# Deci-AI/super-gradients

Measured on NVIDIA H100. Metric: images/sec YOLO-NAS-S 640 bf16 train, higher is better.
Workload: dtype bf16

## Files before the change

include/sgb200.h:

```cpp
#ifndef SGB200_H_
#define SGB200_H_

#include <stdint.h>

#ifdef __cplusplus
extern "C" {
#endif

#define SGB_OK 0
#define SGB_E_INVALID (-1)
#define SGB_E_UNSUPPORTED (-2)
#define SGB_E_CUDA (-3)
#define SGB_E_ARCH (-4)

#define SGB_ACT_NONE 0
#define SGB_ACT_RELU 1
#define SGB_ACT_SILU 2

typedef uint16_t sgb_bf16;

typedef struct SgbConvDesc {
  int32_t N, H, W, C;
  int32_t K, R, S;
  int32_t P, Q;
  int32_t stride, pad;
  int32_t x_pitch, x_off;
  int32_t y_pitch, y_off;
  int32_t up2;
  int32_t centre_from;
} SgbConvDesc;

typedef struct SgbEpilogue {
  const float* scale;
  const float* shift;
  const sgb_bf16* residual;
  double* stats;
  int32_t stats_repl;
  int32_t act;
  int32_t out_f32;
} SgbEpilogue;

const char* sgb_last_error(void);
int sgb_version(void);
int sgb_check_device(void);
int64_t sgb_sm100_launches(void);
int64_t sgb_conv_halo_launches(void);
void sgb_conv_force_im2col(int on);

int sgb_conv_fprop(const SgbConvDesc* d, const sgb_bf16* x, const sgb_bf16* w_krsc, void* y, const SgbEpilogue* ep,
                   void* stream);
int sgb_conv_dgrad(const SgbConvDesc* d, const sgb_bf16* dy, const sgb_bf16* w_crsk, sgb_bf16* dx, int accumulate,
                   void* stream);
int sgb_conv_wgrad(const SgbConvDesc* d, const sgb_bf16* x, const sgb_bf16* dy, float* dw_krsc, void* stream);
int sgb_weight_prepare(const float* w_oihw, int K, int C, int R, int S, int c_pad, sgb_bf16* w_krsc, sgb_bf16* w_crsk,
                       const float* scale, int add_identity, void* stream);
int sgb_wgrad_to_oihw(const float* dw_krsc, int K, int C, int R, int S, int c_pad, float* g_oihw, int accumulate,
                      void* stream);
typedef struct SgbWeightItem {
  const float* w;
  const float* scale;
  sgb_bf16* krsc;
  sgb_bf16* crsk;
  int32_t K, C, R, S, c_pad, add_identity;
  int32_t kp, koff, etaps, etap;
  int64_t start;
} SgbWeightItem;
typedef struct SgbWgradItem {
  const float* dw;
  float* g;
  int32_t K, C, R, S, c_pad, accumulate;
  int64_t start;
} SgbWgradItem;
int sgb_weight_prepare_batch(const SgbWeightItem* items_dev, int n_items, int64_t total, void* stream);
typedef struct SgbAlphaItem {
  const float* dw1;
  const float* w1;
  const float* alpha;
  const float* dab;
  const float* bias1;
  float* g_w1;
  float* g_bias;
  float* g_alpha;
  int32_t K, C, c_pad, pad_;
} SgbAlphaItem;
int sgb_qarep_alpha_finish_batch(const SgbAlphaItem* items_dev, int n_items, void* stream);
int sgb_wgrad_to_oihw_batch(const SgbWgradItem* items_dev, int n_items, int64_t total, void* stream);
int sgb_convt2x2_fprop(const SgbConvDesc* d, const sgb_bf16* x_small, const sgb_bf16* w_up, const float* bias,
                       sgb_bf16* y_up, void* stream);

int sgb_nchw_f32_to_nhwc_bf16(const float* x, int N, int C, int H, int W, sgb_bf16* y, int y_pitch, int y_off, int c_out,
                              void* stream);
int sgb_stem_patches_f32(const float* x, int N, int C, int H, int W, int R, int stride, int pad, sgb_bf16* y, int P, int Q, int c_out,
                         void* stream);
int sgb_nhwc_bf16_to_nchw_f32(const sgb_bf16* x, int N, int C, int H, int W, int x_pitch, int x_off, float* y,
                              void* stream);

typedef struct SgbBnDesc {
  int64_t M;
  int32_t C;
  int32_t x_pitch, x_off;
// ... 305 lines not shown
```

super_gradients_b200/csrc/capi.cu:

```cuda
#include <cstdarg>
#include <cstdio>

#include "common.cuh"
#include "conv_sm100.h"
#include "sm100_host.h"

static thread_local char g_err[512] = "";

void sgb_set_error(const char* fmt, ...) {
  va_list ap;
  va_start(ap, fmt);
  vsnprintf(g_err, sizeof(g_err), fmt, ap);
  va_end(ap);
}

int sgb_cuda_check(cudaError_t e, const char* what) {
  if (e == cudaSuccess) return SGB_OK;
  sgb_set_error("%s: %s", what, cudaGetErrorString(e));
  return SGB_E_CUDA;
}

extern "C" const char* sgb_last_error(void) { return g_err; }
extern "C" int sgb_version(void) { return 100; }
extern "C" int sgb_check_device(void) {
  int dev = 0;
  if (int rc = sgb_cuda_check(cudaGetDevice(&dev), "cudaGetDevice")) return rc;
  cudaDeviceProp prop;
  if (int rc = sgb_cuda_check(cudaGetDeviceProperties(&prop, dev), "cudaGetDeviceProperties")) return rc;
  if (prop.major != 9) {
    sgb_set_error("libsgb200 is built for sm_90a only; device is sm_%d%d", prop.major, prop.minor);
    return SGB_E_ARCH;
  }
  return SGB_OK;
}

extern "C" int64_t sgb_sm100_launches(void) { return (int64_t)sm100::launch_count(); }
extern "C" int64_t sgb_conv_halo_launches(void) { return (int64_t)sm100::halo_launch_count(); }
extern "C" void sgb_conv_force_im2col(int on) { sm100::force_im2col(on != 0); }
```

super_gradients_b200/csrc/conv_sm100.cu:

```cuda
#include <cuda.h>

#include <cstdlib>
#include <cstring>

#include "common.cuh"
#include "conv_sm100.h"
#include "sm100_host.h"
#include "sm100_ptx.cuh"

namespace sm100 {

constexpr int BLOCK_M = 128;
constexpr int NUM_THREADS = 384;
constexpr int CONSUMER_THREADS = 256;
constexpr int MAX_STAGES = 8;

struct Params {
  int M;
  int N;
  int C;
  int KC;
  int n_tiles;
  int stages;
  int P, Q;
// ... 335 lines not shown
      int t = off > 0 ? 0 : CENTRE_TAP;
      uint32_t sa_t = sa + (uint32_t)((t / 3) * HALO_W + t % 3) * 16u, sb_t = sb + (uint32_t)(p.tap_b[t] * ksteps) * b_box;
      for (int k = 0, ks = 0, nk = 8 * off + ksteps; k < nk; ++k) {
        const uint64_t da = smem_desc_noswizzle(sa_t + (uint32_t)(2 * ks) * HALO_CG_BYTES, HALO_CG_BYTES, HALO_W * 16);
        const uint64_t db = smem_desc(sb_t + (uint32_t)ks * b_box, 32, 16u, 256u);
        mma_kk<BN>(acc, da, db, k != 0);
        if (++ks == (t == CENTRE_TAP ? ksteps : off) && ++t < 9) {
          ks = 0;
          sa_t = sa + (uint32_t)((t / 3) * HALO_W + t % 3) * 16u;
          sb_t = sb + (uint32_t)(p.tap_b[t] * ksteps) * b_box;
        }
      }
      wgmma_commit();
      wgmma_wait<0>();
      fence_regs(acc);
      __syncwarp();
      if (lane == 0) mbar_arrive(empty_bar(stg));

      const int n_img = mt / p.halo_thw;
      const int rem = mt - n_img * p.halo_thw;
      const int th = rem / p.halo_tw, tw = rem - th * p.halo_tw;
      const int ow = tw * HALO_TILE + (lane >> 2);
      long long orow[2];
      bool row_ok[2];
#pragma unroll
      for (int h = 0; h < 2; ++h) {
        const int oh = th * HALO_TILE + 2 * wq + h;
        row_ok[h] = oh < p.P && ow < p.Q;
        orow[h] = row_ok[h] ? ((long long)n_img * p.P + oh) * p.Q + ow : 0;
      }
      tile_epilogue<BN, 4>(p, acc, orow, row_ok, nt, wg, wq, lane, s_part + wg * 4 * 2 * BN, s_stats + wg * 2 * p.N);
    }
  }
  __syncthreads();
  if (p.stats) {
    for (int i = threadIdx.x; i < 2 * p.N; i += NUM_THREADS) s_stats[i] += s_stats[2 * p.N + i];
    __syncthreads();
  }
  flush_stats(p, s_stats);
}

struct WParams {
  int K, C;
  int R, S, stride, pad, P, Q;
  int npix;
  int CB;
  int n_ctiles;
  int rb_all, rb_off;
  int items;
  int pix_per_cta;
  int stages;
  int cpad;
  float* dw;
};
constexpr int WPIX = 64;

__host__ __device__ __forceinline__ int wgrad_row_blocks(const WParams& p, int tap) {
  return p.R * p.S == 9 && tap != CENTRE_TAP ? p.rb_off : p.rb_all;
}

template <int NB>
__global__ void __launch_bounds__(NUM_THREADS, 1)
wgrad_wgmma_kernel(const __grid_constant__ CUtensorMap map_dy, const __grid_constant__ CUtensorMap map_x, const WParams p) {
  SGB_GRID_DEP_LAUNCH();
  extern __shared__ __align__(1024) unsigned char smem_raw[];
  const uint32_t smem_base = (smem_u32(smem_raw) + 1023u) & ~1023u;
  const uint32_t a_bytes = 2 * WPIX * 128;
  const uint32_t b_box = WPIX * p.CB * 2;
  const int boxes = NB / p.CB;
  const uint32_t stage_bytes = a_bytes + (uint32_t)boxes * b_box;
  const uint32_t ctrl = smem_base + p.stages * stage_bytes;
  auto full_bar = [&](int s) { return ctrl + 8u * s; };
  auto empty_bar = [&](int s) { return ctrl + 8u * (MAX_STAGES + s); };

  const int warp = threadIdx.x >> 5, lane = threadIdx.x & 31;
  int w = blockIdx.x;
  const int split = w / (p.items * p.n_ctiles);
  w -= split * p.items * p.n_ctiles;
  int tap = 0, tap_items = (wgrad_row_blocks(p, 0) + 1) / 2;
  while (w >= tap_items * p.n_ctiles) {
    w -= tap_items * p.n_ctiles;
    tap_items = (wgrad_row_blocks(p, ++tap) + 1) / 2;
  }
  const int ctile = w / tap_items, item = w - ctile * tap_items;
  const bool shared_rows = 2 * item + 1 == wgrad_row_blocks(p, tap);
  const int row0 = 128 * item;
  const int pix0 = split * p.pix_per_cta;
  const int pix1 = min(pix0 + p.pix_per_cta, p.npix);
  const int n_iters = (pix1 - pix0 + WPIX - 1) / WPIX;

  if (threadIdx.x == 0) {
    for (int s = 0; s < p.stages; ++s) {
      mbar_init(full_bar(s), 1);
      mbar_init(empty_bar(s), shared_rows ? 4 : 8);
    }
    asm volatile("fence.mbarrier_init.release.cluster;" ::: "memory");
    asm volatile("fence.proxy.async.shared::cta;" ::: "memory");
  }
  __syncthreads();
  SGB_GRID_DEP_WAIT();

  if (n_iters > 0) {
    if (warp == 0) {
      if (elect_one()) {
        const int pq = p.P * p.Q;
        const int r = tap / p.S, s = tap - r * p.S;
// ... 18 lines not shown
            par ^= 1;
          }
        }
      }
    } else if (warp >= 4) {
      const int wg = (warp >> 2) - 1, wq = warp & 3;
      const int b_row_bytes = p.CB * 2;
      float acc[NB / 2];
      const int it0 = shared_rows ? wg : 0, it_step = shared_rows ? 2 : 1;
      const uint32_t a_off = shared_rows ? 0u : (uint32_t)wg * (WPIX * 128);
      int stg = it0, prev = -1;
      uint32_t par = 0;
      for (int it = it0; it < n_iters; it += it_step) {
        mbar_wait(full_bar(stg), par);
        const uint32_t sa = smem_base + stg * stage_bytes + a_off, sb = smem_base + stg * stage_bytes + a_bytes;
        wgmma_fence();
#pragma unroll
        for (int j = 0; j < WPIX / 16; ++j) {
          const uint64_t da = smem_desc(sa + (uint32_t)j * 16u * 128u, 128, WPIX * 128, 8 * 128);
          const uint64_t db = smem_desc(sb + (uint32_t)j * 16u * (uint32_t)b_row_bytes, b_row_bytes, b_box, 8u * (uint32_t)b_row_bytes);
          mma_mn<NB>(acc, da, db, (it != it0 || j != 0) ? 1u : 0u);
        }
        wgmma_commit();
        if (prev >= 0) {
          wgmma_wait<1>();
          __syncwarp();
          if (lane == 0) mbar_arrive(empty_bar(prev));
        }
        prev = stg;
        if ((stg += it_step) >= p.stages) {
          stg -= p.stages;
          par ^= 1;
        }
      }
      if (prev < 0) return;
      wgmma_wait<0>();
      fence_regs(acc);
      const int row_len = p.R * p.S * p.cpad;
#pragma unroll
      for (int h = 0; h < 2; ++h) {
        const int ko = row0 + (shared_rows ? 0 : wg * 64) + wq * 16 + (lane >> 2) + 8 * h;
        if (ko < p.K) {
          float* drow = p.dw + (long long)ko * row_len + tap * p.cpad + ctile * NB + 2 * (lane & 3);
#pragma unroll
          for (int j = 0; j < NB / 8; ++j)
            asm volatile("red.global.add.v2.f32 [%0], {%1, %2};" ::"l"(drow + 8 * j), "f"(acc[4 * j + 2 * h]), "f"(acc[4 * j + 2 * h + 1])
                         : "memory");
        }
      }
    }
  }
}

EncodeTiledFn g_tiled = nullptr;
EncodeIm2colFn g_im2col = nullptr;
int g_num_sms = 0;
long long g_launches = 0;
long long g_halo_launches = 0;
bool g_force_im2col = false;
long long launch_count() { return g_launches; }
long long halo_launch_count() { return g_halo_launches; }
void force_im2col(bool on) { g_force_im2col = on; }

int init_driver() {
  if (g_tiled && g_im2col) return SGB_OK;
  cudaDriverEntryPointQueryResult qres;
  void* fn = nullptr;
  if (cudaGetDriverEntryPoint("cuTensorMapEncodeTiled", &fn, cudaEnableDefault, &qres) != cudaSuccess || !fn) {
    sgb_set_error("cuTensorMapEncodeTiled entry point not found");
    return SGB_E_CUDA;
  }
  g_tiled = (EncodeTiledFn)fn;
  fn = nullptr;
  if (cudaGetDriverEntryPoint("cuTensorMapEncodeIm2col", &fn, cudaEnableDefault, &qres) != cudaSuccess || !fn) {
    sgb_set_error("cuTensorMapEncodeIm2col entry point not found");
    return SGB_E_CUDA;
  }
  g_im2col = (EncodeIm2colFn)fn;
  int dev = 0;
  cudaGetDevice(&dev);
  cudaDeviceGetAttribute(&g_num_sms, cudaDevAttrMultiProcessorCount, dev);
  return SGB_OK;
}

CUtensorMapSwizzle swizzle_for(int kc) {
  return kc == 64 ? CU_TENSOR_MAP_SWIZZLE_128B : (kc == 32 ? CU_TENSOR_MAP_SWIZZLE_64B : CU_TENSOR_MAP_SWIZZLE_32B);
}

bool enabled() {
  static int v = -1;
  if (v < 0) {
    const char* e = getenv("SGB_DISABLE_SM100");
    v = (e && e[0] == '1') ? 0 : 1;
  }
  return v == 1;
}

bool supported(const Problem& q) {
  if (!enabled()) return false;
  if (q.C % 16 != 0 || q.b_rows % 8 != 0) return false;
  if (!((q.R == 1 && q.S == 1) || (q.R == 3 && q.S == 3))) return false;
  if (q.stride != 1 && q.stride != 2) return false;
  if (q.a_pitch % 8 != 0 || q.y_pitch % 8 != 0 || q.y_off % 8 != 0) return false;
  if (((uintptr_t)q.a & 15) || ((uintptr_t)q.b & 15) || ((uintptr_t)q.y & 15)) return false;
  if ((long long)q.N * q.P * q.Q >= (1ll << 31)) return false;
  if (q.b_rows > 4096) return false;
  return true;
}

namespace {

template <class Fn>
struct Variant {
  int bn;
  Fn fn;
  int regs;
  bool ready;
};
typedef void (*ConvFn)(const CUtensorMap, const CUtensorMap, const Params);
typedef void (*WgradFn)(const CUtensorMap, const CUtensorMap, const WParams);
Variant<ConvFn> g_conv[] = {{16, conv_wgmma_kernel<16, false>, 0, false},   {32, conv_wgmma_kernel<32, false>, 0, false},
                            {48, conv_wgmma_kernel<48, false>, 0, false},   {64, conv_wgmma_kernel<64, false>, 0, false},
                            {96, conv_wgmma_kernel<96, false>, 0, false},   {128, conv_wgmma_kernel<128, false>, 0, false}};
Variant<ConvFn> g_conv_skip[] = {{16, conv_wgmma_kernel<16, true>, 0, false},   {32, conv_wgmma_kernel<32, true>, 0, false},
                                 {48, conv_wgmma_kernel<48, true>, 0, false},   {64, conv_wgmma_kernel<64, true>, 0, false},
                                 {96, conv_wgmma_kernel<96, true>, 0, false},   {128, conv_wgmma_kernel<128, true>, 0, false}};
Variant<ConvFn> g_halo[] = {{16, conv3x3_halo_kernel<16, false>, 0, false},   {32, conv3x3_halo_kernel<32, false>, 0, false},
                            {48, conv3x3_halo_kernel<48, false>, 0, false},   {64, conv3x3_halo_kernel<64, false>, 0, false},
                            {96, conv3x3_halo_kernel<96, false>, 0, false},   {128, conv3x3_halo_kernel<128, false>, 0, false}};
Variant<ConvFn> g_halo_skip[] = {{16, conv3x3_halo_kernel<16, true>, 0, false},   {32, conv3x3_halo_kernel<32, true>, 0, false},
                                 {48, conv3x3_halo_kernel<48, true>, 0, false},   {64, conv3x3_halo_kernel<64, true>, 0, false},
                                 {96, conv3x3_halo_kernel<96, true>, 0, false},   {128, conv3x3_halo_kernel<128, true>, 0, false}};
Variant<WgradFn> g_wgrad[] = {{16, wgrad_wgmma_kernel<16>, 0, false}, {32, wgrad_wgmma_kernel<32>, 0, false},
                              {48, wgrad_wgmma_kernel<48>, 0, false}, {64, wgrad_wgmma_kernel<64>, 0, false},
                              {96, wgrad_wgmma_kernel<96>, 0, false}, {128, wgrad_wgmma_kernel<128>, 0, false}};

template <class Fn>
int prepare(Variant<Fn>& v, const char* what) {
  if (v.ready) return SGB_OK;
  if (int rc = sgb_cuda_check(cudaFuncSetAttribute(v.fn, cudaFuncAttributeMaxDynamicSharedMemorySize, 227 * 1024), what)) return rc;
  cudaFuncAttributes fa{};
  if (int rc = sgb_cuda_check(cudaFuncGetAttributes(&fa, v.fn), what)) return rc;
  v.regs = fa.numRegs;
  v.ready = true;
  return SGB_OK;
}

int pick_bn(int n) {
  for (int bn : {16, 32, 48, 64, 96, 128})
    if (n <= bn) return bn;
  int best = 128, best_waste = (n + 127) / 128 * 128 - n;
  for (int bn : {96, 64}) {
    const int waste = (n + bn - 1) / bn * bn - n;
    if (waste < best_waste) { best_waste = waste; best = bn; }
  }
  return best;
}

size_t halo_smem(int C, int bn, int n, bool stats, int stages) {
  const size_t b_bytes = ((size_t)9 * C * bn * 2 + 1023) & ~(size_t)1023;
  const size_t a_stage = ((size_t)(C / 8) * HALO_CG_BYTES + 1023) & ~(size_t)1023;
  return 1024 + b_bytes + (size_t)stages * a_stage + HALO_CTRL_BYTES + (stats ? (size_t)(8 * 2 * bn + 4 * n) * 4 : 0);
}

int halo_bn(const Problem& q) {
  if (q.R != 3 || q.S != 3 || q.stride != 1 || q.pad != 1 || q.ntaps > 0 || q.out_mode != 0) return 0;
  if (q.P != q.H || q.Q != q.W) return 0;
  const long long covered = (long long)((q.P + 7) / 8) * 8 * ((q.Q + 7) / 8) * 8;
  if (20ll * q.P * q.Q < 17 * covered) return 0;
  const int n = q.b_rows, full = pick_bn(n);
  auto waste = [&](int bn) { return (n + bn - 1) / bn * bn - n; };
  for (int bn : {full, 96, 64})
    if (bn <= full && (bn == full || (q.C <= 96 && bn >= 64 && waste(bn) <= waste(full))) &&
        halo_smem(q.C, bn, n, q.stats != nullptr, 2) <= 227 * 1024)
      return bn;
  return 0;
}

int launch_halo(const Problem& q, const Params& p0, int bn, cudaStream_t st) {
  Params p = p0;
  p.n_tiles = (p.N + bn - 1) / bn;
  p.halo_tw = (q.Q + HALO_TILE - 1) / HALO_TILE;
  p.halo_thw = p.halo_tw * ((q.P + HALO_TILE - 1) / HALO_TILE);
  p.M = q.N * p.halo_thw;
  p.centre_n = 0;
  Variant<ConvFn>* var = nullptr;
  for (auto& v : p.centre_c > 0 ? g_halo_skip : g_halo)
    if (v.bn == bn) var = &v;
  if (int rc = prepare(*var, "conv3x3_halo_kernel")) return rc;
  const int regs_alloc = ((var->regs + 7) / 8) * 8 * NUM_THREADS;
  int ctas_per_sm = 65536 / regs_alloc;
  if (ctas_per_sm > 2) ctas_per_sm = 2;
  if (ctas_per_sm < 1) ctas_per_sm = 1;
  int stages = 0;
  for (;; --ctas_per_sm) {
    const size_t budget = (ctas_per_sm == 1 ? 227u : 227u / ctas_per_sm - 1u) * 1024u;
    for (stages = HALO_MAX_STAGES; stages >= 2 && halo_smem(q.C, bn, p.N, p.stats != nullptr, stages) > budget; --stages) {
    }
    if (stages >= 2 || ctas_per_sm == 1) break;
  }
  if (stages < 2) { sgb_set_error("conv3x3_halo: tile does not fit shared memory"); return SGB_E_UNSUPPORTED; }
  p.stages = stages;
  const size_t smem = halo_smem(q.C, bn, p.N, p.stats != nullptr, stages);

  alignas(64) CUtensorMap map_a, map_b;
  {
    cuuint64_t dims[4] = {(cuuint64_t)q.C, (cuuint64_t)q.W, (cuuint64_t)q.H, (cuuint64_t)q.N};
    cuuint64_t strides[3] = {(cuuint64_t)q.a_pitch * 2, (cuuint64_t)q.W * q.a_pitch * 2, (cuuint64_t)q.H * q.W * q.a_pitch * 2};
    cuuint32_t box[4] = {8, HALO_W, HALO_H, 1};
    cuuint32_t estr[4] = {1, 1, 1, 1};
    CUresult r = g_tiled(&map_a, CU_TENSOR_MAP_DATA_TYPE_BFLOAT16, 4, const_cast<void*>(q.a), dims, strides, box, estr,
                         CU_TENSOR_MAP_INTERLEAVE_NONE, CU_TENSOR_MAP_SWIZZLE_NONE, CU_TENSOR_MAP_L2_PROMOTION_L2_128B,
                         CU_TENSOR_MAP_FLOAT_OOB_FILL_NONE);
    if (r != CUDA_SUCCESS) {
      sgb_set_error("cuTensorMapEncodeTiled(halo) failed with %d (C=%d W=%d H=%d N=%d pitch=%d)", (int)r, q.C, q.W, q.H, q.N, q.a_pitch);
      return SGB_E_CUDA;
    }
  }
  {
    cuuint64_t dims[2] = {(cuuint64_t)q.b_cols, (cuuint64_t)q.b_rows};
    cuuint64_t strides[1] = {(cuuint64_t)q.b_cols * 2};
    cuuint32_t box[2] = {16, (cuuint32_t)bn};
    cuuint32_t estr[2] = {1, 1};
    CUresult r = g_tiled(&map_b, CU_TENSOR_MAP_DATA_TYPE_BFLOAT16, 2, const_cast<void*>(q.b), dims, strides, box, estr,
                         CU_TENSOR_MAP_INTERLEAVE_NONE, CU_TENSOR_MAP_SWIZZLE_32B, CU_TENSOR_MAP_L2_PROMOTION_L2_128B,
                         CU_TENSOR_MAP_FLOAT_OOB_FILL_NONE);
    if (r != CUDA_SUCCESS) {
      sgb_set_error("cuTensorMapEncodeTiled(halo B) failed with %d (cols=%d rows=%d BN=%d)", (int)r, q.b_cols, q.b_rows, bn);
      return SGB_E_CUDA;
    }
  }
  int per_nt = g_num_sms * ctas_per_sm / p.n_tiles;
  if (per_nt > p.M) per_nt = p.M;
  if (per_nt < 1) per_nt = 1;
  SGB_LAUNCH(var->fn, per_nt * p.n_tiles, NUM_THREADS, smem, st, map_a, map_b, p);
  ++g_launches;
  ++g_halo_launches;
  return sgb_cuda_check(cudaGetLastError(), "conv3x3_halo_kernel");
}

}

int launch(const Problem& q, cudaStream_t st) {
  if (int rc = init_driver()) return rc;
  Params p{};
  p.M = q.N * q.P * q.Q;
  p.N = q.b_rows;
  p.C = q.C;
  p.KC = q.C % 64 == 0 ? 64 : (q.C % 32 == 0 ? 32 : 16);
  if (p.KC < 64 && q.C > 32) p.KC = 64;
  const int bn = pick_bn(p.N);
  p.n_tiles = (p.N + bn - 1) / bn;
  p.P = q.P; p.Q = q.Q; p.stride = q.stride; p.pad = q.pad;
  if (q.ntaps > 0) {
    p.ntaps = q.ntaps;
    for (int t = 0; t < q.ntaps; ++t) { p.tap_dh[t] = (signed char)q.tap_dh[t]; p.tap_dw[t] = (signed char)q.tap_dw[t]; p.tap_b[t] = (signed char)q.tap_b[t]; }
  } else {
    p.ntaps = q.R * q.S;
    for (int t = 0; t < p.ntaps; ++t) {
      p.tap_dh[t] = (signed char)(t / q.S);
      p.tap_dw[t] = (signed char)(t % q.S);
      p.tap_b[t] = (signed char)(q.flip ? (p.ntaps - 1 - t) : t);
    }
  }
  if (p.ntaps > 9) return SGB_E_UNSUPPORTED;
  p.out_mode = q.out_mode; p.o_mul = q.o_mul; p.oh_add = q.oh_add; p.ow_add = q.ow_add; p.outH = q.outH; p.outW = q.outW;
  p.b_cols_per_tap = q.b_cols_per_tap;
  p.y = (bf16*)q.y; p.y_pitch = q.y_pitch; p.y_off = q.y_off;
  p.scale = q.scale; p.shift = q.shift; p.residual = (const bf16*)q.residual;
  p.stats = q.stats; p.stats_repl = q.stats_repl > 0 ? q.stats_repl : 1; p.act = q.act;
  if (q.centre_from > 0) {
// ... 29 lines not shown
  alignas(64) CUtensorMap map_a, map_b;
  {
    cuuint64_t dims[4] = {(cuuint64_t)q.C, (cuuint64_t)q.W, (cuuint64_t)q.H, (cuuint64_t)q.N};
    cuuint64_t strides[3] = {(cuuint64_t)q.a_pitch * 2, (cuuint64_t)q.W * q.a_pitch * 2, (cuuint64_t)q.H * q.W * q.a_pitch * 2};
    int lower[2] = {-q.pad, -q.pad};
    int upper[2] = {q.pad - (q.S - 1), q.pad - (q.R - 1)};
    if (q.ntaps > 0) {
      lower[0] = lower[1] = 0;
      upper[0] = q.Q - q.W;
      upper[1] = q.P - q.H;
    }
    cuuint32_t estr[4] = {1, (cuuint32_t)q.stride, (cuuint32_t)q.stride, 1};
    CUresult r = g_im2col(&map_a, CU_TENSOR_MAP_DATA_TYPE_BFLOAT16, 4, const_cast<void*>(q.a), dims, strides, lower, upper,
                          (cuuint32_t)p.KC, (cuuint32_t)BLOCK_M, estr, CU_TENSOR_MAP_INTERLEAVE_NONE, swizzle_for(p.KC),
                          CU_TENSOR_MAP_L2_PROMOTION_L2_128B, CU_TENSOR_MAP_FLOAT_OOB_FILL_NONE);
    if (r != CUDA_SUCCESS) {
      sgb_set_error("cuTensorMapEncodeIm2col failed with %d (C=%d W=%d H=%d N=%d pitch=%d pad=%d upper=%d,%d stride=%d KC=%d)", (int)r,
                    q.C, q.W, q.H, q.N, q.a_pitch, q.pad, upper[0], upper[1], q.stride, p.KC);
      return SGB_E_CUDA;
    }
  }
  {
    cuuint64_t dims[2] = {(cuuint64_t)q.b_cols, (cuuint64_t)q.b_rows};
    cuuint64_t strides[1] = {(cuuint64_t)q.b_cols * 2};
    cuuint32_t box[2] = {(cuuint32_t)p.KC, (cuuint32_t)bn};
    cuuint32_t estr[2] = {1, 1};
    CUresult r = g_tiled(&map_b, CU_TENSOR_MAP_DATA_TYPE_BFLOAT16, 2, const_cast<void*>(q.b), dims, strides, box, estr,
                         CU_TENSOR_MAP_INTERLEAVE_NONE, swizzle_for(p.KC), CU_TENSOR_MAP_L2_PROMOTION_L2_128B,
                         CU_TENSOR_MAP_FLOAT_OOB_FILL_NONE);
    if (r != CUDA_SUCCESS) {
      sgb_set_error("cuTensorMapEncodeTiled(B) failed with %d (cols=%d rows=%d KC=%d BN=%d)", (int)r, q.b_cols, q.b_rows, p.KC, bn);
      return SGB_E_CUDA;
    }
  }
  const int m_tiles = (p.M + BLOCK_M - 1) / BLOCK_M;
  int grid = m_tiles * p.n_tiles;
  if (grid > g_num_sms * ctas_per_sm) grid = g_num_sms * ctas_per_sm;
  SGB_LAUNCH(var->fn, grid, NUM_THREADS, smem, st, map_a, map_b, p);
  ++g_launches;
  return sgb_cuda_check(cudaGetLastError(), "conv_wgmma_kernel");
}

bool wgrad_supported(const WgradProblem& q) {
  if (!enabled()) return false;
  if (q.C % 16 != 0 || q.K % 8 != 0) return false;
  if (!((q.R == 1 && q.S == 1) || (q.R == 3 && q.S == 3))) return false;
  if (q.pad != q.R / 2 || (q.stride != 1 && q.stride != 2)) return false;
  if (q.x_pitch % 8 != 0 || q.y_pitch % 8 != 0) return false;
  if (((uintptr_t)q.x & 15) || ((uintptr_t)q.dy & 15)) return false;
  if ((long long)q.N * q.P * q.Q >= (1ll << 31)) return false;
  return true;
}

int wgrad_launch(const WgradProblem& q, cudaStream_t st) {
  if (int rc = init_driver()) return rc;
  WParams p{};
  p.K = q.K; p.C = q.C; p.R = q.R; p.S = q.S; p.stride = q.stride; p.pad = q.pad; p.P = q.P; p.Q = q.Q;
  p.npix = q.N * q.P * q.Q;
  int nb = 16;
  for (int cand : {128, 96, 64, 48, 32})
    if (q.C % cand == 0) { nb = cand; break; }
  p.CB = nb % 64 == 0 ? 64 : (nb % 32 == 0 ? 32 : 16);
  p.n_ctiles = q.C / nb;
  if (q.centre_from != 0 && (q.R != 3 || q.S != 3 || q.stride != 1 || q.pad != 1 || q.centre_from < 0 || q.centre_from >= q.K ||
                             q.centre_from % 16 != 0))
    return SGB_E_INVALID;
  p.rb_all = (q.K + 63) / 64;
  p.rb_off = q.centre_from > 0 ? (q.centre_from + 63) / 64 : p.rb_all;
  p.items = 0;
  for (int t = 0; t < q.R * q.S; ++t) p.items += (wgrad_row_blocks(p, t) + 1) / 2;
  p.cpad = q.C;
  p.dw = q.dw;
  Variant<WgradFn>* var = nullptr;
  for (auto& v : g_wgrad)
    if (v.bn == nb) var = &v;
  if (int rc = prepare(*var, "wgrad_wgmma_kernel")) return rc;
  const uint32_t stage_bytes = 2 * WPIX * 128 + (uint32_t)(nb / p.CB) * WPIX * p.CB * 2;
  int stages = (int)((200 * 1024 - CTRL_BAR_BYTES - 1024) / stage_bytes);
  if (stages > MAX_STAGES) stages = MAX_STAGES;
  if (p.rb_all % 2 || p.rb_off % 2) stages &= ~1;
  if (stages < 2) return SGB_E_UNSUPPORTED;
  p.stages = stages;
  const size_t smem = 1024 + (size_t)stages * stage_bytes + CTRL_BAR_BYTES;
  const int base_ctas = p.items * p.n_ctiles;
  const int total_iters = (p.npix + WPIX - 1) / WPIX;
  int splits = (2 * g_num_sms + base_ctas - 1) / base_ctas;
  if (splits > total_iters / 8) splits = total_iters / 8;
  if (splits < 1) splits = 1;
  int iters_per = (total_iters + splits - 1) / splits;
  p.pix_per_cta = iters_per * WPIX;
  splits = (p.npix + p.pix_per_cta - 1) / p.pix_per_cta;

  alignas(64) CUtensorMap map_dy, map_x;
  {
    cuuint64_t dims[2] = {(cuuint64_t)q.K, (cuuint64_t)p.npix};
    cuuint64_t strides[1] = {(cuuint64_t)q.y_pitch * 2};
    cuuint32_t box[2] = {64, (cuuint32_t)WPIX};
    cuuint32_t estr[2] = {1, 1};
    CUresult r = g_tiled(&map_dy, CU_TENSOR_MAP_DATA_TYPE_BFLOAT16, 2, const_cast<void*>(q.dy), dims, strides, box, estr,
                         CU_TENSOR_MAP_INTERLEAVE_NONE, CU_TENSOR_MAP_SWIZZLE_128B, CU_TENSOR_MAP_L2_PROMOTION_L2_128B,
                         CU_TENSOR_MAP_FLOAT_OOB_FILL_NONE);
    if (r != CUDA_SUCCESS) { sgb_set_error("cuTensorMapEncodeTiled(dy) failed with %d", (int)r); return SGB_E_CUDA; }
  }
  {
    cuuint64_t dims[4] = {(cuuint64_t)q.C, (cuuint64_t)q.W, (cuuint64_t)q.H, (cuuint64_t)q.N};
    cuuint64_t strides[3] = {(cuuint64_t)q.x_pitch * 2, (cuuint64_t)q.W * q.x_pitch * 2, (cuuint64_t)q.H * q.W * q.x_pitch * 2};
    int lower[2] = {-q.pad, -q.pad};
    int upper[2] = {q.pad - (q.S - 1), q.pad - (q.R - 1)};
    cuuint32_t estr[4] = {1, (cuuint32_t)q.stride, (cuuint32_t)q.stride, 1};
    CUresult r = g_im2col(&map_x, CU_TENSOR_MAP_DATA_TYPE_BFLOAT16, 4, const_cast<void*>(q.x), dims, strides, lower, upper,
                          (cuuint32_t)p.CB, (cuuint32_t)WPIX, estr, CU_TENSOR_MAP_INTERLEAVE_NONE,
                          swizzle_for(p.CB), CU_TENSOR_MAP_L2_PROMOTION_L2_128B,
                          CU_TENSOR_MAP_FLOAT_OOB_FILL_NONE);
    if (r != CUDA_SUCCESS) { sgb_set_error("cuTensorMapEncodeIm2col(x, wgrad) failed with %d", (int)r); return SGB_E_CUDA; }
  }
  const int grid = base_ctas * splits;
  SGB_LAUNCH(var->fn, grid, NUM_THREADS, smem, st, map_dy, map_x, p);
  ++g_launches;
  return sgb_cuda_check(cudaGetLastError(), "wgrad_wgmma_kernel");
}

}
```

super_gradients_b200/csrc/conv_sm100.h:

```cpp
#pragma once
#include <cuda_runtime.h>

namespace sm100 {

struct Problem {
  const void* a;
  int N, H, W, C, a_pitch;
  const void* b;
  int b_rows, b_cols, b_cols_per_tap;
  int R, S, stride, pad, P, Q, flip;
  int ntaps;
  int tap_dh[9], tap_dw[9], tap_b[9];
  int out_mode, o_mul, oh_add, ow_add, outH, outW;
  void* y;
  int y_pitch, y_off;
  const float* scale;
  const float* shift;
  const void* residual;
  double* stats;
  int stats_repl, act;
  int centre_from;
};

struct WgradProblem {
  const void* x;
  const void* dy;
  int N, H, W, C, x_pitch;
  int K, y_pitch;
  int R, S, stride, pad, P, Q;
  float* dw;
  int centre_from;
};

bool enabled();
bool wgrad_supported(const WgradProblem& q);
int wgrad_launch(const WgradProblem& q, cudaStream_t st);
bool supported(const Problem& q);
int launch(const Problem& q, cudaStream_t st);
long long launch_count();
long long halo_launch_count();
void force_im2col(bool on);

}
```

super_gradients_b200/lib.py:

```python
import ctypes
import os
from ctypes import POINTER, Structure, c_char_p, c_double, c_float, c_int, c_int32, c_int64, c_void_p

_HERE = os.path.dirname(os.path.abspath(__file__))
LIB_PATH = os.environ.get("SGB200_LIB") or os.path.join(_HERE, "libsgb200.so")

ACT_NONE, ACT_RELU, ACT_SILU = 0, 1, 2


class SgbError(RuntimeError):
    pass


class ConvDesc(Structure):
    _fields_ = [(n, c_int32) for n in ("N", "H", "W", "C", "K", "R", "S", "P", "Q", "stride", "pad", "x_pitch", "x_off", "y_pitch", "y_off", "up2", "centre_from")]


class Epilogue(Structure):
    _fields_ = [
        ("scale", c_void_p),
        ("shift", c_void_p),
        ("residual", c_void_p),
        ("stats", c_void_p),
        ("stats_repl", c_int32),
# ... 81 lines not shown
class PreprocDesc(Structure):
    _fields_ = (
        [(n, c_int32) for n in ("src_h", "src_w", "src_c", "src_pitch", "dst_h", "dst_w", "out_h", "out_w", "pad_top", "pad_left", "out_pitch", "reverse_channels", "normalize")]
        + [("pad_value", c_float), ("max_value", c_double), ("mean", c_float * 4), ("std", c_float * 4)]
    )


class MatchDesc(Structure):
    _fields_ = [(n, c_int32) for n in ("B", "max_preds", "max_targets", "max_crowd", "n_thresholds", "top_k", "denormalize_targets")] + [("height", c_float), ("width", c_float)]


class LossDesc(Structure):
    _fields_ = [
        ("B", c_int32),
        ("L", c_int32),
        ("ncls", c_int32),
        ("reg_max", c_int32),
        ("n_max", c_int32),
        ("topk", c_int32),
        ("alpha", c_float),
        ("beta", c_float),
        ("w_cls", c_float),
        ("w_iou", c_float),
        ("w_dfl", c_float),
        ("iou_type", c_int32),
    ]


class NmsDesc(Structure):
    _fields_ = [
        ("B", c_int32),
        ("L", c_int32),
        ("ncls", c_int32),
        ("score_thr", c_float),
        ("iou_thr", c_double),
        ("top_k", c_int32),
        ("max_out", c_int32),
        ("multi_label", c_int32),
        ("class_agnostic", c_int32),
        ("thr_inclusive", c_int32),
    ]


P = c_void_p
_I, _F, _L = c_int, c_float, c_int64

_SIGNATURES = {
    "sgb_last_error": (c_char_p, []),
    "sgb_version": (c_int, []),
    "sgb_check_device": (c_int, []),
    "sgb_sm100_launches": (c_int64, []),
    "sgb_conv_halo_launches": (c_int64, []),
    "sgb_conv_force_im2col": (None, [_I]),
    "sgb_conv_fprop": (c_int, [POINTER(ConvDesc), P, P, P, POINTER(Epilogue), P]),
    "sgb_conv_dgrad": (c_int, [POINTER(ConvDesc), P, P, P, _I, P]),
    "sgb_conv_wgrad": (c_int, [POINTER(ConvDesc), P, P, P, P]),
    "sgb_weight_prepare": (c_int, [P, _I, _I, _I, _I, _I, P, P, P, _I, P]),
    "sgb_wgrad_to_oihw": (c_int, [P, _I, _I, _I, _I, _I, P, _I, P]),
    "sgb_weight_prepare_batch": (c_int, [P, _I, c_int64, P]),
    "sgb_wgrad_to_oihw_batch": (c_int, [P, _I, c_int64, P]),
    "sgb_qarep_alpha_finish_batch": (c_int, [P, _I, P]),
    "sgb_convt2x2_fprop": (c_int, [POINTER(ConvDesc), P, P, P, P, P]),
    "sgb_nchw_f32_to_nhwc_bf16": (c_int, [P, _I, _I, _I, _I, P, _I, _I, _I, P]),
    "sgb_stem_patches_f32": (c_int, [P, _I, _I, _I, _I, _I, _I, _I, P, _I, _I, _I, P]),
    "sgb_nhwc_bf16_to_nchw_f32": (c_int, [P, _I, _I, _I, _I, _I, _I, P, P]),
    "sgb_bn_act_fwd": (c_int, [POINTER(BnDesc), P, P, P, P, P, P, P, P, P, P, P]),
    "sgb_bn_act_fwd_fused": (c_int, [POINTER(BnDesc), P, P, P, P, P, P, P, P, P, P, P]),
    "sgb_bn_act_infer": (c_int, [POINTER(BnDesc), P, P, P, P, P, P, P, P]),
    "sgb_bn_act_bwd_reduce": (c_int, [POINTER(BnDesc), P, P, P, P, P, P, P, P, P]),
    "sgb_bn_act_bwd_apply": (c_int, [POINTER(BnDesc), P, P, P, P, P, P, P, P, P, P, P, P, P]),
    "sgb_bn_act_bwd_fused": (c_int, [POINTER(BnDesc), P, P, P, P, P, P, P, P, P, P, P, P, P]),
    "sgb_channel_stats": (c_int, [P, _L, _I, _I, _I, P, P]),
    "sgb_qarep_moments": (c_int, [POINTER(QarepDesc), P, P, P, P]),
    "sgb_qarep_fwd": (c_int, [POINTER(QarepDesc)] + [P] * 15),
    "sgb_qarep_fwd_fused": (c_int, [POINTER(QarepDesc)] + [P] * 15),
    "sgb_qarep_bwd_reduce": (c_int, [POINTER(QarepDesc), P, P, P, P, P, P, P]),
    "sgb_qarep_bwd_apply": (c_int, [POINTER(QarepDesc)] + [P] * 16),
    "sgb_qarep_bwd_fused": (c_int, [POINTER(QarepDesc)] + [P] * 15),
    "sgb_maxpool_fwd": (c_int, [P, _I, _I, _I, _I, _I, _I, _I, _I, _I, P, _I, _I, _I, _I, P, P]),
    "sgb_maxpool_bwd": (c_int, [P, _I, _I, _I, _I, _I, _I, _I, _I, _I, _I, _I, P, P, P]),
    "sgb_maxpool_bwd_bf16": (c_int, [P, _I, _I, _I, _I, _I, _I, _I, _I, _I, _I, _I, P, P, _I, P]),
    "sgb_axpby": (c_int, [P, _I, _I, _F, P, _I, _I, _F, P, _I, _I, _L, _I, P]),
    "sgb_scale_add": (c_int, [P, _I, _I, P, P, _I, _I, P, _I, _I, _L, _I, P]),
    "sgb_channel_dot": (c_int, [P, _I, _I, P, _I, _I, _L, _I, P, P]),
    "sgb_scale_add_dot": (c_int, [P, _I, _I, P, P, _I, _I, P, _I, _I, P, _I, _I, _L, _I, P, P]),
    "sgb_f32_to_bf16": (c_int, [P, P, _L, P]),
    "sgb_avgpool_fwd": (c_int, [P, _I, _I, _I, P, P]),
    "sgb_avgpool_bwd": (c_int, [P, _I, _I, _I, P, P]),
    "sgb_dfl_decode": (c_int, [P, _I, P, _I, _I, _I, _I, _I, _I, _I, _I, _F, _F, P, P, P, P, P]),
    "sgb_pose_keypoint_decode": (c_int, [P, _I, P, _I, _I, _I, _I, _I, _I, _I, _I, _F, _F, _F, _I, P, P, P, P]),
    "sgb_tal_assign": (c_int, [POINTER(LossDesc)] + [P] * 12 + [_L, P]),
    "sgb_tal_workspace_bytes": (c_int64, [POINTER(LossDesc)]),
    "sgb_atss_assign": (c_int, [POINTER(LossDesc)] + [P] * 5 + [c_int32] + [P] * 7 + [P, _L, P]),
    "sgb_atss_workspace_bytes": (c_int64, [POINTER(LossDesc)]),
    "sgb_dfl_iou_loss_fwd_bwd": (c_int, [POINTER(LossDesc)] + [P] * 8 + [_F, P, P, P]),
    "sgb_focal_cls_fwd_bwd": (c_int, [POINTER(LossDesc), P, P, P, P, c_float, c_float, P, P]),
    "sgb_loss_finalize": (c_int, [POINTER(LossDesc), P, P, P]),
    "sgb_preprocess_u8": (c_int, [POINTER(PreprocDesc), P, P, P]),
    "sgb_resample_crop_u8": (c_int, [P, P, P, _L, _I, _I, _I, _I, _I, _I, c_double, P, P, P, P]),
    "sgb_classify_rows": (c_int, [P, _L, _I, _L, _I, P, P, _L, _I, _I, P, P, P, P]),
    "sgb_detection_augment": (c_int, [P, P, P, _L, _I, _I, _I, _I, _I, _I, c_double, _I, P, P]),
    "sgb_pose_augment": (c_int, [P, P, P, _L, P, _L, _I, _I, _I, c_double, _I, P, P]),
    "sgb_detection_matching": (c_int, [POINTER(MatchDesc), P, P, P, P, P, P, P, P, P, P]),
    "sgb_pose_keypoint_matching": (c_int, [P] * 10 + [_I] * 6 + [P] * 7),
    "sgb_pose_tal_workspace_bytes": (c_int64, [POINTER(PoseLossDesc)]),
    "sgb_pose_tal_assign": (c_int, [POINTER(PoseLossDesc)] + [P] * 14 + [_L, P]),
    "sgb_pose_loss_fwd_bwd": (c_int, [POINTER(PoseLossDesc)] + [P] * 12 + [_F] + [P] * 5),
    "sgb_pose_loss_finalize": (c_int, [POINTER(PoseLossDesc), P, P, P]),
    "sgb_head_grad_scatter": (c_int, [P, _I, _I, _I, _I, _I, P, _I, P]),
    "sgb_sliding_window_gather": (c_int, [P, _I, _I, _I, _I, P, P, _I, _I, P, P]),
    "sgb_sliding_window_merge_workspace_bytes": (c_int64, [_I, P, _I, _I, _I]),
    "sgb_sliding_window_merge": (c_int, [P, P, P, P, P, _I, _I, _I, _I, c_double, P, P, P, _L, P]),
    "sgb_sliding_window_merge_launches": (c_int32, [_I, P, _I, _I]),
    "sgb_nms_workspace_bytes": (c_int64, [POINTER(NmsDesc)]),
    "sgb_batched_nms": (c_int, [POINTER(NmsDesc), P, P, P, P, P, P, _L, P]),
    "sgb_sgd_step": (c_int, [P, P, P, _L, P, P]),
    "sgb_adamw_step": (c_int, [P, P, P, P, _L, P, P]),
    "sgb_ema_update": (c_int, [P, P, _L, P, P]),
}

_lib = None

LAUNCH_COUNT = {"sgb_tal_assign": 4, "sgb_atss_assign": 3, "sgb_pose_tal_assign": 4, "sgb_sm100_launches": 0, "sgb_conv_halo_launches": 0, "sgb_conv_force_im2col": 0, "sgb_sliding_window_merge_workspace_bytes": 0, "sgb_sliding_window_merge_launches": 0, "sgb_last_error": 0, "sgb_version": 0, "sgb_check_device": 0}
LAUNCHES = [0]


def exported_names():
    return sorted(_SIGNATURES)


def load():
    global _lib
    if _lib is not None:
        return _lib
    if not os.path.exists(LIB_PATH):
        raise SgbError(f"{LIB_PATH} not found: run `python -c 'import __graft_entry__ as g; g.build()'` " "(there is no non-CUDA fallback for this package)")
    lib = ctypes.CDLL(LIB_PATH)
    for name, (res, args) in _SIGNATURES.items():
        fn = getattr(lib, name)
        fn.restype = res
        fn.argtypes = args
    _lib = lib
    return lib


def check(rc, what=""):
    if rc != 0:
        msg = load().sgb_last_error()
        raise SgbError(f"{what} failed with code {rc}: {msg.decode() if msg else ''}")


def call(name, *args):
    lib = load()
    rc = getattr(lib, name)(*args)
    LAUNCHES[0] += LAUNCH_COUNT.get(name, 1)
    if rc != 0:
        msg = lib.sgb_last_error()
        raise SgbError(f"{name} failed with code {rc}: {msg.decode() if msg else ''}")
```

Measured before the change: 915.5.

## Add halo-tiled 3x3 stride-1 wgrad kernel reusing one x tile for all taps

Adds a dedicated weight-gradient kernel for 3x3, stride-1, pad-1 convolutions. Each stage loads an 8x8 dy tile and a single haloed x tile by TMA, and the nine taps are computed by offsetting smem descriptors into that tile. This replaces the per-tap im2col loads of the generic wgrad kernel. Taps are split across the two consumer warpgroups (5/4, or centre-only for the off rows) with fp32 red.add outputs. It is enabled by default when the spatial tiles fit, with a force-im2col switch and launch counter for fallback. Risks include load imbalance between warpgroups and idle warpgroups on the centre-only row blocks.

```diff
diff --git a/include/sgb200.h b/include/sgb200.h
--- a/include/sgb200.h
+++ b/include/sgb200.h
@@ -46,6 +46,8 @@
 int64_t sgb_sm100_launches(void);
 int64_t sgb_conv_halo_launches(void);
 void sgb_conv_force_im2col(int on);
+int64_t sgb_conv_wgrad_halo_launches(void);
+void sgb_conv_wgrad_force_im2col(int on);
 
 int sgb_conv_fprop(const SgbConvDesc* d, const sgb_bf16* x, const sgb_bf16* w_krsc, void* y, const SgbEpilogue* ep,
                    void* stream);
diff --git a/super_gradients_b200/csrc/capi.cu b/super_gradients_b200/csrc/capi.cu
--- a/super_gradients_b200/csrc/capi.cu
+++ b/super_gradients_b200/csrc/capi.cu
@@ -37,3 +37,5 @@
 extern "C" int64_t sgb_sm100_launches(void) { return (int64_t)sm100::launch_count(); }
 extern "C" int64_t sgb_conv_halo_launches(void) { return (int64_t)sm100::halo_launch_count(); }
 extern "C" void sgb_conv_force_im2col(int on) { sm100::force_im2col(on != 0); }
+extern "C" int64_t sgb_conv_wgrad_halo_launches(void) { return (int64_t)sm100::wgrad_halo_launch_count(); }
+extern "C" void sgb_conv_wgrad_force_im2col(int on) { sm100::wgrad_force_im2col(on != 0); }
diff --git a/super_gradients_b200/csrc/conv_sm100.cu b/super_gradients_b200/csrc/conv_sm100.cu
--- a/super_gradients_b200/csrc/conv_sm100.cu
+++ b/super_gradients_b200/csrc/conv_sm100.cu
@@ -411,6 +411,7 @@
   int stages;
   int cpad;
   float* dw;
+  int halo_tw, halo_thw, tiles, tiles_per_cta;
 };
 constexpr int WPIX = 64;
 
@@ -535,15 +536,153 @@
   }
 }
 
+constexpr uint32_t WH_A_BYTES = WPIX * 128;
+
+__host__ __device__ constexpr uint32_t wgrad_halo_stage_bytes(int nb) {
+  return (WH_A_BYTES + (uint32_t)(nb / 8) * HALO_CG_BYTES + 1023u) & ~1023u;
+}
+
+template <int NB, int NT>
+__device__ __forceinline__ void wgrad_halo_consume(const WParams& p, uint32_t ring, uint32_t bars, int t0, int t1, int tap0, int rb,
+                                                   int ctile) {
+  constexpr uint32_t stage_bytes = wgrad_halo_stage_bytes(NB);
+  const int wq = (threadIdx.x >> 5) & 3, lane = threadIdx.x & 31;
+  auto full_bar = [&](int s) { return bars + 8u * s; };
+  auto empty_bar = [&](int s) { return bars + 8u * (MAX_STAGES + s); };
+  float acc[NT > 0 ? NT : 1][NB / 2];
+  int stg = 0, prev = 0;
+  uint32_t par = 0;
+  for (int mt = t0; mt < t1; ++mt) {
+    mbar_wait(full_bar(stg), par);
+    if constexpr (NT > 0) {
+      const uint32_t sa = ring + stg * stage_bytes, sx = sa + WH_A_BYTES;
+      wgmma_fence();
+#pragma unroll
+      for (int t = 0; t < NT; ++t) {
+        const int tap = tap0 + t;
+        const uint32_t sx_t = sx + (uint32_t)((tap / 3) * HALO_W + tap % 3) * 16u;
+#pragma unroll
+        for (int j = 0; j < WPIX / 16; ++j) {
+          const uint64_t da = smem_desc(sa + (uint32_t)j * 16u * 128u, 128, WPIX * 128, 8 * 128);
+          const uint64_t db = smem_desc_noswizzle(sx_t + (uint32_t)j * 2u * HALO_W * 16u, HALO_W * 16, HALO_CG_BYTES);
+          mma_mn<NB>(acc[t], da, db, (mt != t0 || j != 0) ? 1u : 0u);
+        }
+      }
+      wgmma_commit();
+      wgmma_wait<1>();
+    }
+    __syncwarp();
+    if (lane == 0 && mt != t0) mbar_arrive(empty_bar(prev));
+    prev = stg;
+    if (++stg == p.stages) {
+      stg = 0;
+      par ^= 1;
+    }
+  }
+  if constexpr (NT > 0) {
+    wgmma_wait<0>();
+#pragma unroll
+    for (int t = 0; t < NT; ++t) fence_regs(acc[t]);
+  }
+  __syncwarp();
+  if (lane == 0) mbar_arrive(empty_bar(prev));
+  if constexpr (NT > 0) {
+    const int row_len = 9 * p.cpad;
+#pragma unroll
+    for (int h = 0; h < 2; ++h) {
+      const int ko = 64 * rb + wq * 16 + (lane >> 2) + 8 * h;
+      if (ko < p.K) {
+        float* drow = p.dw + (long long)ko * row_len + tap0 * p.cpad + ctile * NB + 2 * (lane & 3);
+#pragma unroll
+        for (int t = 0; t < NT; ++t)
+#pragma unroll
+          for (int j = 0; j < NB / 8; ++j)
+            asm volatile("red.global.add.v2.f32 [%0], {%1, %2};" ::"l"(drow + t * p.cpad + 8 * j), "f"(acc[t][4 * j + 2 * h]),
+                         "f"(acc[t][4 * j + 2 * h + 1])
+                         : "memory");
+      }
+    }
+  }
+}
+
+template <int NB>
+__global__ void __launch_bounds__(NUM_THREADS, 1)
+wgrad3x3_halo_kernel(const __grid_constant__ CUtensorMap map_dy, const __grid_constant__ CUtensorMap map_x, const WParams p) {
+  SGB_GRID_DEP_LAUNCH();
+  extern __shared__ __align__(1024) unsigned char smem_raw[];
+  const uint32_t smem_base = (smem_u32(smem_raw) + 1023u) & ~1023u;
+  constexpr uint32_t a_bytes = WH_A_BYTES, stage_bytes = wgrad_halo_stage_bytes(NB);
+  const uint32_t ctrl = smem_base + p.stages * stage_bytes;
+  auto full_bar = [&](int s) { return ctrl + 8u * s; };
+  auto empty_bar = [&](int s) { return ctrl + 8u * (MAX_STAGES + s); };
+
+  const int warp = threadIdx.x >> 5;
+  const int items = p.rb_all * p.n_ctiles;
+  const int split = blockIdx.x / items, item = blockIdx.x - split * items;
+  const int ctile = item / p.rb_all, rb = item - ctile * p.rb_all;
+  const bool all_taps = rb < p.rb_off;
+  const int t0 = split * p.tiles_per_cta, t1 = min(t0 + p.tiles_per_cta, p.tiles);
+
+  if (threadIdx.x == 0) {
+    for (int s = 0; s < p.stages; ++s) {
+      mbar_init(full_bar(s), 1);
+      mbar_init(empty_bar(s), 8);
+    }
+    asm volatile("fence.mbarrier_init.release.cluster;" ::: "memory");
+    asm volatile("fence.proxy.async.shared::cta;" ::: "memory");
+  }
+  __syncthreads();
+  SGB_GRID_DEP_WAIT();
+
+  if (warp == 0) {
+    if (elect_one()) {
+      const uint32_t tx = a_bytes + (NB / 8) * (HALO_H * HALO_W * 16);
+      int stg = 0;
+      uint32_t par = 1;
+      for (int mt = t0; mt < t1; ++mt) {
+        const int n_img = mt / p.halo_thw;
+        const int rem = mt - n_img * p.halo_thw;
+        const int th = rem / p.halo_tw, tw = rem - th * p.halo_tw;
+        mbar_wait(empty_bar(stg), par);
+        const uint32_t sa = smem_base + stg * stage_bytes;
+        mbar_expect_tx(full_bar(stg), tx);
+        tma_load_tiled_4d(sa, &map_dy, full_bar(stg), 64 * rb, tw * HALO_TILE, th * HALO_TILE, n_img);
+        for (int cg = 0; cg < NB / 8; ++cg)
+          tma_load_tiled_4d(sa + a_bytes + (uint32_t)cg * HALO_CG_BYTES, &map_x, full_bar(stg), ctile * NB + 8 * cg,
+                            tw * HALO_TILE - 1, th * HALO_TILE - 1, n_img);
+        if (++stg == p.stages) {
+          stg = 0;
+          par ^= 1;
+        }
+      }
+    }
+  } else if (warp >= 4) {
+    const int wg = (warp >> 2) - 1;
+    const uint32_t ring = smem_base, bars = ctrl;
+    if (!all_taps && wg == 0)
+      wgrad_halo_consume<NB, 1>(p, ring, bars, t0, t1, CENTRE_TAP, rb, ctile);
+    else if (!all_taps)
+      wgrad_halo_consume<NB, 0>(p, ring, bars, t0, t1, 0, rb, ctile);
+    else if (wg == 0)
+      wgrad_halo_consume<NB, 5>(p, ring, bars, t0, t1, 0, rb, ctile);
+    else
+      wgrad_halo_consume<NB, 4>(p, ring, bars, t0, t1, 5, rb, ctile);
+  }
+}
+
 EncodeTiledFn g_tiled = nullptr;
 EncodeIm2colFn g_im2col = nullptr;
 int g_num_sms = 0;
 long long g_launches = 0;
 long long g_halo_launches = 0;
+long long g_wgrad_halo_launches = 0;
 bool g_force_im2col = false;
+bool g_wgrad_force_im2col = false;
 long long launch_count() { return g_launches; }
 long long halo_launch_count() { return g_halo_launches; }
+long long wgrad_halo_launch_count() { return g_wgrad_halo_launches; }
 void force_im2col(bool on) { g_force_im2col = on; }
+void wgrad_force_im2col(bool on) { g_wgrad_force_im2col = on; }
 
 int init_driver() {
   if (g_tiled && g_im2col) return SGB_OK;
@@ -617,6 +756,8 @@
 Variant<WgradFn> g_wgrad[] = {{16, wgrad_wgmma_kernel<16>, 0, false}, {32, wgrad_wgmma_kernel<32>, 0, false},
                               {48, wgrad_wgmma_kernel<48>, 0, false}, {64, wgrad_wgmma_kernel<64>, 0, false},
                               {96, wgrad_wgmma_kernel<96>, 0, false}, {128, wgrad_wgmma_kernel<128>, 0, false}};
+Variant<WgradFn> g_wgrad_halo[] = {{16, wgrad3x3_halo_kernel<16>, 0, false}, {32, wgrad3x3_halo_kernel<32>, 0, false},
+                                   {48, wgrad3x3_halo_kernel<48>, 0, false}};
 
 template <class Fn>
 int prepare(Variant<Fn>& v, const char* what) {
@@ -646,11 +787,15 @@
   return 1024 + b_bytes + (size_t)stages * a_stage + HALO_CTRL_BYTES + (stats ? (size_t)(8 * 2 * bn + 4 * n) * 4 : 0);
 }
 
+bool halo_tiles_fit(int P, int Q) {
+  const long long covered = (long long)((P + 7) / 8) * 8 * ((Q + 7) / 8) * 8;
+  return 20ll * P * Q >= 17 * covered;
+}
+
 int halo_bn(const Problem& q) {
   if (q.R != 3 || q.S != 3 || q.stride != 1 || q.pad != 1 || q.ntaps > 0 || q.out_mode != 0) return 0;
   if (q.P != q.H || q.Q != q.W) return 0;
-  const long long covered = (long long)((q.P + 7) / 8) * 8 * ((q.Q + 7) / 8) * 8;
-  if (20ll * q.P * q.Q < 17 * covered) return 0;
+  if (!halo_tiles_fit(q.P, q.Q)) return 0;
   const int n = q.b_rows, full = pick_bn(n);
   auto waste = [&](int bn) { return (n + bn - 1) / bn * bn - n; };
   for (int bn : {full, 96, 64})
@@ -658,6 +803,20 @@
         halo_smem(q.C, bn, n, q.stats != nullptr, 2) <= 227 * 1024)
       return bn;
   return 0;
+}
+
+int encode_halo_map(CUtensorMap* map, const void* x, int N, int H, int W, int C, int pitch) {
+  cuuint64_t dims[4] = {(cuuint64_t)C, (cuuint64_t)W, (cuuint64_t)H, (cuuint64_t)N};
+  cuuint64_t strides[3] = {(cuuint64_t)pitch * 2, (cuuint64_t)W * pitch * 2, (cuuint64_t)H * W * pitch * 2};
+  cuuint32_t box[4] = {8, HALO_W, HALO_H, 1};
+  cuuint32_t estr[4] = {1, 1, 1, 1};
+  CUresult r = g_tiled(map, CU_TENSOR_MAP_DATA_TYPE_BFLOAT16, 4, const_cast<void*>(x), dims, strides, box, estr, CU_TENSOR_MAP_INTERLEAVE_NONE,
+                       CU_TENSOR_MAP_SWIZZLE_NONE, CU_TENSOR_MAP_L2_PROMOTION_L2_128B, CU_TENSOR_MAP_FLOAT_OOB_FILL_NONE);
+  if (r != CUDA_SUCCESS) {
+    sgb_set_error("cuTensorMapEncodeTiled(halo) failed with %d (C=%d W=%d H=%d N=%d pitch=%d)", (int)r, C, W, H, N, pitch);
+    return SGB_E_CUDA;
+  }
+  return SGB_OK;
 }
 
 int launch_halo(const Problem& q, const Params& p0, int bn, cudaStream_t st) {
@@ -687,19 +846,7 @@
   const size_t smem = halo_smem(q.C, bn, p.N, p.stats != nullptr, stages);
 
   alignas(64) CUtensorMap map_a, map_b;
-  {
-    cuuint64_t dims[4] = {(cuuint64_t)q.C, (cuuint64_t)q.W, (cuuint64_t)q.H, (cuuint64_t)q.N};
-    cuuint64_t strides[3] = {(cuuint64_t)q.a_pitch * 2, (cuuint64_t)q.W * q.a_pitch * 2, (cuuint64_t)q.H * q.W * q.a_pitch * 2};
-    cuuint32_t box[4] = {8, HALO_W, HALO_H, 1};
-    cuuint32_t estr[4] = {1, 1, 1, 1};
-    CUresult r = g_tiled(&map_a, CU_TENSOR_MAP_DATA_TYPE_BFLOAT16, 4, const_cast<void*>(q.a), dims, strides, box, estr,
-                         CU_TENSOR_MAP_INTERLEAVE_NONE, CU_TENSOR_MAP_SWIZZLE_NONE, CU_TENSOR_MAP_L2_PROMOTION_L2_128B,
-                         CU_TENSOR_MAP_FLOAT_OOB_FILL_NONE);
-    if (r != CUDA_SUCCESS) {
-      sgb_set_error("cuTensorMapEncodeTiled(halo) failed with %d (C=%d W=%d H=%d N=%d pitch=%d)", (int)r, q.C, q.W, q.H, q.N, q.a_pitch);
-      return SGB_E_CUDA;
-    }
-  }
+  if (int rc = encode_halo_map(&map_a, q.a, q.N, q.H, q.W, q.C, q.a_pitch)) return rc;
   {
     cuuint64_t dims[2] = {(cuuint64_t)q.b_cols, (cuuint64_t)q.b_rows};
     cuuint64_t strides[1] = {(cuuint64_t)q.b_cols * 2};
@@ -835,6 +982,59 @@
   return true;
 }
 
+namespace {
+
+int wgrad_halo_nb(const WgradProblem& q) {
+  if (q.R != 3 || q.S != 3 || q.stride != 1 || q.pad != 1 || q.P != q.H || q.Q != q.W) return 0;
+  if (!halo_tiles_fit(q.P, q.Q)) return 0;
+  return q.C % 32 == 0 ? 32 : (q.C % 48 == 0 ? 48 : 16);
+}
+
+int launch_wgrad_halo(const WgradProblem& q, const WParams& p0, int nb, cudaStream_t st) {
+  WParams p = p0;
+  p.n_ctiles = q.C / nb;
+  p.halo_tw = (q.Q + HALO_TILE - 1) / HALO_TILE;
+  p.halo_thw = p.halo_tw * ((q.P + HALO_TILE - 1) / HALO_TILE);
+  p.tiles = q.N * p.halo_thw;
+  Variant<WgradFn>* var = nullptr;
+  for (auto& v : g_wgrad_halo)
+    if (v.bn == nb) var = &v;
+  if (int rc = prepare(*var, "wgrad3x3_halo_kernel")) return rc;
+  const int ctas_per_sm = ((var->regs + 7) / 8) * 8 * NUM_THREADS * 2 <= 65536 ? 2 : 1;
+  const uint32_t stage_bytes = wgrad_halo_stage_bytes(nb);
+  const uint32_t budget = (ctas_per_sm == 1 ? 227u : 113u) * 1024u - 1024u - CTRL_BAR_BYTES;
+  p.stages = (int)(budget / stage_bytes);
+  if (p.stages > MAX_STAGES) p.stages = MAX_STAGES;
+  const size_t smem = 1024 + (size_t)p.stages * stage_bytes + CTRL_BAR_BYTES;
+  const int items = p.rb_all * p.n_ctiles;
+  int splits = g_num_sms * ctas_per_sm / items;
+  if (splits < 1) splits = 1;
+  p.tiles_per_cta = (p.tiles + splits - 1) / splits;
+  splits = (p.tiles + p.tiles_per_cta - 1) / p.tiles_per_cta;
+
+  alignas(64) CUtensorMap map_dy, map_x;
+  {
+    cuuint64_t dims[4] = {(cuuint64_t)q.K, (cuuint64_t)q.Q, (cuuint64_t)q.P, (cuuint64_t)q.N};
+    cuuint64_t strides[3] = {(cuuint64_t)q.y_pitch * 2, (cuuint64_t)q.Q * q.y_pitch * 2, (cuuint64_t)q.P * q.Q * q.y_pitch * 2};
+    cuuint32_t box[4] = {64, HALO_TILE, HALO_TILE, 1};
+    cuuint32_t estr[4] = {1, 1, 1, 1};
+    CUresult r = g_tiled(&map_dy, CU_TENSOR_MAP_DATA_TYPE_BFLOAT16, 4, const_cast<void*>(q.dy), dims, strides, box, estr,
+                         CU_TENSOR_MAP_INTERLEAVE_NONE, CU_TENSOR_MAP_SWIZZLE_128B, CU_TENSOR_MAP_L2_PROMOTION_L2_128B,
+                         CU_TENSOR_MAP_FLOAT_OOB_FILL_NONE);
+    if (r != CUDA_SUCCESS) {
+      sgb_set_error("cuTensorMapEncodeTiled(dy tile) failed with %d (K=%d Q=%d P=%d N=%d pitch=%d)", (int)r, q.K, q.Q, q.P, q.N, q.y_pitch);
+      return SGB_E_CUDA;
+    }
+  }
+  if (int rc = encode_halo_map(&map_x, q.x, q.N, q.H, q.W, q.C, q.x_pitch)) return rc;
+  SGB_LAUNCH(var->fn, splits * items, NUM_THREADS, smem, st, map_dy, map_x, p);
+  ++g_launches;
+  ++g_wgrad_halo_launches;
+  return sgb_cuda_check(cudaGetLastError(), "wgrad3x3_halo_kernel");
+}
+
+}
+
 int wgrad_launch(const WgradProblem& q, cudaStream_t st) {
   if (int rc = init_driver()) return rc;
   WParams p{};
@@ -854,6 +1054,8 @@
   for (int t = 0; t < q.R * q.S; ++t) p.items += (wgrad_row_blocks(p, t) + 1) / 2;
   p.cpad = q.C;
   p.dw = q.dw;
+  if (!g_wgrad_force_im2col)
+    if (const int nb = wgrad_halo_nb(q)) return launch_wgrad_halo(q, p, nb, st);
   Variant<WgradFn>* var = nullptr;
   for (auto& v : g_wgrad)
     if (v.bn == nb) var = &v;
diff --git a/super_gradients_b200/csrc/conv_sm100.h b/super_gradients_b200/csrc/conv_sm100.h
--- a/super_gradients_b200/csrc/conv_sm100.h
+++ b/super_gradients_b200/csrc/conv_sm100.h
@@ -40,5 +40,7 @@
 long long launch_count();
 long long halo_launch_count();
 void force_im2col(bool on);
+long long wgrad_halo_launch_count();
+void wgrad_force_im2col(bool on);
 
 }
diff --git a/super_gradients_b200/lib.py b/super_gradients_b200/lib.py
--- a/super_gradients_b200/lib.py
+++ b/super_gradients_b200/lib.py
@@ -157,6 +157,8 @@
     "sgb_sm100_launches": (c_int64, []),
     "sgb_conv_halo_launches": (c_int64, []),
     "sgb_conv_force_im2col": (None, [_I]),
+    "sgb_conv_wgrad_halo_launches": (c_int64, []),
+    "sgb_conv_wgrad_force_im2col": (None, [_I]),
     "sgb_conv_fprop": (c_int, [POINTER(ConvDesc), P, P, P, POINTER(Epilogue), P]),
     "sgb_conv_dgrad": (c_int, [POINTER(ConvDesc), P, P, P, _I, P]),
     "sgb_conv_wgrad": (c_int, [POINTER(ConvDesc), P, P, P, P]),
@@ -226,7 +228,7 @@
 
 _lib = None
 
-LAUNCH_COUNT = {"sgb_tal_assign": 4, "sgb_atss_assign": 3, "sgb_pose_tal_assign": 4, "sgb_sm100_launches": 0, "sgb_conv_halo_launches": 0, "sgb_conv_force_im2col": 0, "sgb_sliding_window_merge_workspace_bytes": 0, "sgb_sliding_window_merge_launches": 0, "sgb_last_error": 0, "sgb_version": 0, "sgb_check_device": 0}
+LAUNCH_COUNT = {"sgb_tal_assign": 4, "sgb_atss_assign": 3, "sgb_pose_tal_assign": 4, "sgb_sm100_launches": 0, "sgb_conv_halo_launches": 0, "sgb_conv_force_im2col": 0, "sgb_conv_wgrad_halo_launches": 0, "sgb_conv_wgrad_force_im2col": 0, "sgb_sliding_window_merge_workspace_bytes": 0, "sgb_sliding_window_merge_launches": 0, "sgb_last_error": 0, "sgb_version": 0, "sgb_check_device": 0}
 LAUNCHES = [0]
 
 
```

New measurement: 955.7, median of 6. 1.04x the previous value.
